# Dizzy-cell/HOUV

Measured on AMD Instinct MI355X. Metric: registration pairs/sec (2048-pt partial pairs), higher is better.
Workload: dtype f32; 1 GPU; HOUV solve_model, 2048x2048-pt pairs, batch 256/GPU, K=64 restarts x 200 Adam iterations + retry stages (BASELINE configs[1]); pairs_per_gpu=256, points=2048, kernel=64, iters=200, icp_refine=False, parallelism=dp1 (pair shards, one RCCL all-gather of [steps*P,12] per rank)

## Files before the change

houv_amd/_lib.py:

```python
import ctypes
import os

import torch

_HERE = os.path.dirname(os.path.abspath(__file__))
LIB_PATH = os.environ.get("HOUV_HIP_LIB") or os.path.join(_HERE, "lib", "libhouv_hip.so")
ABI_VERSION = 2

_c_f = ctypes.c_void_p
_int = ctypes.c_int
_dbl = ctypes.c_double
_flt = ctypes.c_float

_SIGNATURES = {
    "houv_abi_version": (ctypes.c_int, []),
    "houv_last_error": (ctypes.c_char_p, []),
    "houv_build_id": (ctypes.c_char_p, []),
    "houv_debug_set": (ctypes.c_int, [ctypes.c_char_p, ctypes.c_longlong]),
    "houv_chamfer_forward": (ctypes.c_int, [_c_f, _c_f, _int, _int, _int, _c_f, _c_f, _c_f, _c_f, _c_f]),
    "houv_chamfer_backward": (ctypes.c_int, [_c_f, _c_f, _int, _int, _int, _c_f, _c_f, _c_f, _c_f, _c_f, _c_f, _c_f]),
    "houv_kabsch": (ctypes.c_int, [_c_f, _c_f, _c_f, _int, _int, _c_f, _c_f, _c_f]),
    "houv_solve_iterate": (ctypes.c_int, [_c_f, _c_f, _int, _int, _int, _int, _c_f, _int, _int, _int, _int, _int, _int,
                                          _int, _int, _dbl, _dbl, _dbl, _dbl, _flt, _c_f, _c_f, _c_f, _c_f, _c_f, _c_f,
                                          _c_f]),
    "houv_solve_iterate_large": (ctypes.c_int, [_c_f, _c_f, _int, _int, _int, _int, _c_f, _int, _int, _int, _int, _int, _int,
                                                _int, _int, _dbl, _dbl, _dbl, _dbl, _flt, _c_f, _c_f, _c_f, _c_f, _c_f, _c_f,
                                                _c_f]),
    "houv_solve_iterate_pruned": (ctypes.c_int, [_c_f, _c_f, _int, _int, _int, _int, _c_f, _int, _int, _int, _int, _int,
                                                 _int, _int, _int, _dbl, _dbl, _dbl, _dbl, _flt, _c_f, _c_f, _c_f, _c_f,
                                                 _c_f, _c_f, _c_f, _int, _int, _c_f]),
    "houv_solve_variant": (ctypes.c_int, [_int, _int, _int, ctypes.POINTER(ctypes.c_int), ctypes.POINTER(ctypes.c_int),
                                          ctypes.POINTER(ctypes.c_int)]),
    "houv_solve_lds_bytes": (ctypes.c_longlong, [_int, _int, _int]),
    "houv_kd_sort": (ctypes.c_int, [_c_f, _int, _int, _int, _int, _c_f, _c_f, _c_f]),
    "houv_icp_refine": (ctypes.c_int, [_c_f, _c_f, _int, _int, _int, _c_f, _flt, _int, _flt, _flt, _c_f, _c_f, _c_f, _c_f, _c_f]),
    "houv_knn": (ctypes.c_int, [_c_f, _int, _int, _int, _c_f, _c_f]),
    "houv_edgeconv1": (ctypes.c_int, [_c_f, _c_f, _int, _int, _int, _c_f, _c_f, _c_f, _c_f, _c_f]),
    "houv_max_over_k": (ctypes.c_int, [_c_f, ctypes.c_longlong, _int, _int, _c_f, _int, _c_f]),
    "houv_gemm_f32": (ctypes.c_int, [_c_f, _c_f, _c_f, _int, _int, _int, _int, _int, _int, _int, _int, _int] +
                      [ctypes.c_longlong] * 6 + [_flt, _c_f, _c_f, _c_f, _int, ctypes.c_longlong, ctypes.c_longlong,
                                                 _int, _c_f]),
    "houv_attention_f32": (ctypes.c_int, [_c_f, _c_f, _c_f, _c_f, _int, _int, _int, _int, _int, _int, _int, _int, _int] +
                           [ctypes.c_longlong] * 4 + [_flt, _c_f]),
    "houv_layernorm": (ctypes.c_int, [_c_f, ctypes.c_longlong, _int, _c_f, _c_f, _flt, _c_f, _c_f, _c_f]),
    "houv_softmax_rows": (ctypes.c_int, [_c_f, ctypes.c_longlong, _int, _c_f]),
    "houv_softmax_corr": (ctypes.c_int, [_c_f, _int, _int, _int, _c_f, _c_f, _c_f]),
    "houv_furthest_point_sample": (ctypes.c_int, [_c_f, _int, _int, _int, _c_f, _c_f]),
    "houv_knn_cross": (ctypes.c_int, [_c_f, _c_f, _int, _int, _int, _int, _c_f, _c_f, _c_f]),
# ... 41 lines not shown
        fn.restype = res
        fn.argtypes = args
    if lib.houv_abi_version() != ABI_VERSION:
        raise HouvHipError(f"libhouv_hip.so ABI {lib.houv_abi_version()} != expected {ABI_VERSION}")
    _lib = lib
    return lib


def solve_variant(N, M, pruned=False, with_mode=False):
    b, q, m = ctypes.c_int(0), ctypes.c_int(0), ctypes.c_int(0)
    check(load().houv_solve_variant(int(N), int(M), int(bool(pruned)), ctypes.byref(b), ctypes.byref(q), ctypes.byref(m)),
          "houv_solve_variant")
    return (b.value, q.value, m.value) if with_mode else (b.value, q.value)


def build_id():
    return load().houv_build_id().decode()


def debug_set(name, value):
    check(load().houv_debug_set(name.encode(), int(value)), "houv_debug_set")


def last_error():
    return load().houv_last_error().decode("utf-8", "replace")


def check(ok, what):
    if ok != 1:
        raise HouvHipError(f"{what} failed: {last_error()}")
# ... 33 lines not shown
```

houv_amd/csrc/capi.hip:

```cpp
#include <stdarg.h>
#include <string.h>

#include "../../include/houv_hip.h"
#include "houv_common.h"

namespace houv {

static thread_local char g_err[512] = "";

void set_error(const char* fmt, ...) {
  va_list ap;
  va_start(ap, fmt);
  vsnprintf(g_err, sizeof(g_err), fmt, ap);
  va_end(ap);
  fprintf(stderr, "[houv_hip] %s\n", g_err);
}

DebugKnobs g_debug;

namespace {

__global__ void pose_kernel(const float* __restrict__ params, int n, int angle_base, int trans_mode,
                            float* __restrict__ R, float* __restrict__ T) {
  const int i = blockIdx.x * blockDim.x + threadIdx.x;
// ... 25 lines not shown
}

extern "C" int houv_abi_version(void) { return HOUV_ABI_VERSION; }

extern "C" const char* houv_last_error(void) { return houv::g_err; }

extern "C" int houv_debug_set(const char* name, long long value) {
  using namespace houv;
  const struct { const char* name; std::atomic<int>* knob; long long lo, hi, step; } ints[] = {
      {"solve_predict", &g_debug.pred_mode, 0, 2, 1}, {"knn_split", &g_debug.knn_split, 0, 1, 1},
      {"attn_split", &g_debug.attn_split, 0, 1, 1},   {"gemm_split", &g_debug.gemm_split, 0, 6, 3}};
  if (name && !strcmp(name, "solve_stats")) {
    g_debug.stats = (unsigned long long)value;
    return 1;
  }
  for (const auto& k : ints)
    if (name && !strcmp(name, k.name) && value >= k.lo && value <= k.hi && value % k.step == 0) {
      *k.knob = (int)value;
      return 1;
    }
  set_error("houv_debug_set: unknown switch or value out of range: %s = %lld", name ? name : "(null)", value);
  return 0;
}

#ifndef HOUV_BUILD_ID
#define HOUV_BUILD_ID "unknown"
#endif
extern "C" const char* houv_build_id(void) { return HOUV_BUILD_ID; }

extern "C" int houv_pose_forward(const float* params, int n, int angle_base, int trans_mode, const float* src, int N,
// ... 18 lines not shown
```

houv_amd/csrc/houv_common.h:

```cpp
#pragma once
#include <hip/hip_runtime.h>
#include <stdint.h>
#include <stdio.h>

#include <atomic>

#include "houv_math.h"

namespace houv {

constexpr int kWave = 64;
constexpr int kSub = 32;
constexpr int kTrk = 16;

void set_error(const char* fmt, ...);
struct SolveCommon;
__attribute__((visibility("hidden"))) int solve_check_args(const char* who, const SolveCommon& a, int use_views);
inline bool check_launch(const char* what) {
  hipError_t e = hipGetLastError();
  if (e != hipSuccess) {
    set_error("%s: %s", what, hipGetErrorString(e));
    return false;
  }
  return true;
}

struct DebugKnobs {
  std::atomic<int> pred_mode{0};
  std::atomic<unsigned long long> stats{0ull};
  std::atomic<int> knn_split{1};
  std::atomic<int> attn_split{1};
  std::atomic<int> gemm_split{6};
};
extern DebugKnobs g_debug;

template <int MET>
__device__ __forceinline__ float metric_sqdist(float dx, float dy, float dz) {
  if constexpr (MET == 0) return __builtin_fmaf(dz, dz, __builtin_fmaf(dy, dy, dx * dx));
  else if constexpr (MET == 1) return __builtin_fmaf(dz, dz, dy * dy);
  else if constexpr (MET == 2) return __builtin_fmaf(dz, dz, dx * dx);
  else return __builtin_fmaf(dy, dy, dx * dx);
}

__device__ __forceinline__ float min3f(float a, float b, float c) {
// ... 67 lines not shown
```

houv_amd/csrc/houv_math.h:

```cpp
#pragma once
#include <math.h>

#if defined(__HIPCC__)
#define HOUV_HD __host__ __device__
#else
#define HOUV_HD
#endif

namespace houv {

constexpr float kPiF = 3.14159274101257324f;

enum TransMode { kTransHouv = 0, kTransSolve = 1 };

HOUV_HD inline float tsqrt(float x) { return sqrtf(x); }
HOUV_HD inline double tsqrt(double x) { return sqrt(x); }

struct Pose {
  float R[9];
  float T[3];
  float u[3], inv_vnorm, sin_t, cos_t, chat[3], inv_cnorm, sigma, a, s;
};

HOUV_HD inline void pose_forward(const float p[8], int angle_base, int trans_mode, Pose& o) {
// ... 222 lines not shown
#pragma unroll
    for (int i = 0; i < 3; ++i) Ts[i] = stale[(m * 12 + 9 + i) * stride];
    term_travel(Rs, Ts, R, T, def_now, radius, d_s, t_s);
    const bool s0 = (stale_bits >> m) & 1u, s1 = (stale_bits >> (4 + m)) & 1u;
    const float d0 = s0 ? d_s : d_f, d1 = s1 ? d_s : d_f;
    const float t0 = s0 ? t_s : t_f, t1 = s1 ? t_s : t_f;
    const float c0 = cd[2 * m], c1 = cd[2 * m + 1];
    const float dd = d0 + d1;
    const float slack = dd + kTermRel * (fabsf(c0) + fabsf(c1) + dd) + kTermAbs +
                        kTermMoveErr * (2.0f * radius + tn + 0.5f * (t0 + t1));
    const unsigned drop1 = (c0 + slack < c1) ? (0x10u << m) : 0u;
    const unsigned drop0 = (c1 + slack < c0) ? (1u << m) : 0u;
    need &= ~(drop0 | drop1);
  }
  return need;
}

template <typename T>
HOUV_HD inline void svd3x3(const T H[9], T U[9], T S[3], T V[9]) {
  T B[9];
  for (int i = 0; i < 9; ++i) { B[i] = H[i]; V[i] = (i % 4 == 0) ? (T)1 : (T)0; }
  const int P[3] = {0, 0, 1}, Qi[3] = {1, 2, 2};
  for (int sweep = 0; sweep < 12; ++sweep) {
    T off = 0;
    for (int r = 0; r < 3; ++r) {
      const int p = P[r], q = Qi[r];
      const T a = B[0 * 3 + p] * B[0 * 3 + p] + B[1 * 3 + p] * B[1 * 3 + p] + B[2 * 3 + p] * B[2 * 3 + p];
      const T b = B[0 * 3 + q] * B[0 * 3 + q] + B[1 * 3 + q] * B[1 * 3 + q] + B[2 * 3 + q] * B[2 * 3 + q];
      const T g = B[0 * 3 + p] * B[0 * 3 + q] + B[1 * 3 + p] * B[1 * 3 + q] + B[2 * 3 + p] * B[2 * 3 + q];
      const T eps2 = sizeof(T) == 4 ? (T)1e-14 : (T)1e-31;
// ... 74 lines not shown
```

houv_amd/csrc/houv_sweep.h:

```cpp
#pragma once
#include "houv_common.h"

namespace houv {

typedef float houv_f4v __attribute__((ext_vector_type(4)));
typedef const houv_f4v __attribute__((address_space(3))) * lds_f4;

__device__ __forceinline__ int tid_x() {
  int t = threadIdx.x;
  asm volatile("" : "+v"(t));
  return t;
}
typedef __amdgpu_buffer_rsrc_t buf_t;
__device__ __forceinline__ buf_t make_buf(const void* base, int bytes) {
  return __builtin_amdgcn_make_buffer_rsrc(const_cast<void*>(base), (short)0, bytes, 0x00020000);
}

template <int Q, int NMET>
__device__ __forceinline__ void sweep_tile(const float4* __restrict__ rp, const float (&qx)[Q], const float (&qy)[Q],
                                           const float (&qz)[Q], const float (&in)[Q][NMET], float (&out)[Q][NMET]) {
#pragma unroll
  for (int j = 0; j < kTrk; j += 2) {
    const float4 a = rp[j], c = rp[j + 1];
    asm volatile("" ::"v"(a.w), "v"(c.w));
// ... 170 lines not shown

constexpr int kNnRec = 8;

__device__ __forceinline__ unsigned select_mask(unsigned long long lanes, unsigned a, unsigned b) {
  unsigned r;
  asm("v_cndmask_b32_e64 %0, %1, %2, %3" : "=v"(r) : "v"(a), "v"(b), "s"(lanes));
  return r;
}

__device__ __forceinline__ unsigned lowest_bit_or_m1(unsigned x) {
  unsigned r;
  asm("v_ffbl_b32_e32 %0, %1" : "=v"(r) : "v"(x));
  return r;
}

template <int NMET>
__device__ __forceinline__ void gather_tile_min(unsigned xa, float cx, float cy, float cz, const float (&cb)[NMET],
                                                float (&ta)[NMET], float (&tb)[NMET]) {
  constexpr int kBatch = 4, kHalf = kSub / 2;
  static_assert(kSub == 32 && kHalf == kTrk, "two 256-B tracking units of 16 slots");
  auto fetch = [&](float4 (&r)[kBatch], int i0) {
#pragma unroll
    for (int u = 0; u < kBatch; u += 2) {
      lds_f4 p = (lds_f4)(size_t)(xa ^ ((unsigned)((i0 + u / 2) & (kHalf - 1)) << 4));
      const houv_f4v v0 = p[0], v1 = p[kHalf];
      r[u] = make_float4(v0.x, v0.y, v0.z, v0.w);
      r[u + 1] = make_float4(v1.x, v1.y, v1.z, v1.w);
    }
  };
  auto eval2 = [&](const float4 a, const float4 c, const float (&in)[NMET], float (&t)[NMET]) {
    const float ax = a.x - cx, ay = a.y - cy, az = a.z - cz;
    const float bx = c.x - cx, by = c.y - cy, bz = c.z - cz;
    if constexpr (NMET == 4) {
      const float axx = ax * ax, ayy = ay * ay, bxx = bx * bx, byy = by * by;
      const float a3 = __builtin_fmaf(ay, ay, axx), b3 = __builtin_fmaf(by, by, bxx);
      const float a1 = __builtin_fmaf(az, az, ayy), b1 = __builtin_fmaf(bz, bz, byy);
      const float a2 = __builtin_fmaf(az, az, axx), b2 = __builtin_fmaf(bz, bz, bxx);
      const float a0 = __builtin_fmaf(az, az, a3), b0 = __builtin_fmaf(bz, bz, b3);
      t[0] = min3f(in[0], a0, b0);
      t[1] = min3f(in[1], a1, b1);
      t[2] = min3f(in[2], a2, b2);
      t[3] = min3f(in[3], a3, b3);
    } else {
      t[0] = min3f(in[0], metric_sqdist<0>(ax, ay, az), metric_sqdist<0>(bx, by, bz));
    }
  };
  float inf[NMET];
#pragma unroll
  for (int m = 0; m < NMET; ++m) inf[m] = INFINITY;
  auto eval = [&](float4 (&r)[kBatch], bool first) {
#pragma unroll
    for (int u = 0; u < kBatch; ++u) asm volatile("" ::"v"(r[u].x), "v"(r[u].y), "v"(r[u].z), "v"(r[u].w));
    static_assert(kBatch == 4, "a batch = two slots x two units");
    if (first) {
      eval2(r[0], r[2], cb, ta);
      eval2(r[1], r[3], inf, tb);
    } else {
      eval2(r[0], r[2], ta, ta);
      eval2(r[1], r[3], tb, tb);
    }
  };
  float4 ra[kBatch], rb[kBatch];
  fetch(ra, 0);
#pragma unroll
  for (int i0 = 0; i0 < kHalf; i0 += kBatch) {
    fetch(rb, i0 + kBatch / 2);
    eval(ra, i0 == 0);
    if (i0 + kBatch < kHalf) fetch(ra, i0 + kBatch);
    eval(rb, false);
  }
}

__device__ __forceinline__ void take_units(float ta, float tb, int unit0, float& cb, int& ct) {
  const unsigned long long la = __builtin_amdgcn_ballot_w64(ta < cb), lb = __builtin_amdgcn_ballot_w64(tb < ta);
  ct = (int)select_mask(lb, select_mask(la, (unsigned)ct, (unsigned)unit0), (unsigned)unit0 + 1u);
  cb = __uint_as_float(select_mask(lb, __float_as_uint(ta), __float_as_uint(tb)));
}

template <int BLOCK, int Q, int NMET>
__device__ __forceinline__ void prune_masks(const float4* __restrict__ refs, const float4* __restrict__ boxes, int ntile,
                                            const float (&qx)[Q], const float (&qy)[Q], const float (&qz)[Q],
                                            buf_t ws, int prev_off, int count, unsigned need,
                                            unsigned long long (&un)[Q]) {
  float ub[Q][NMET];
#pragma unroll
  for (int k = 0; k < Q; ++k) {
    const bool ok = pt_index<BLOCK>(k) < count;
    unsigned w0 = 0u, w1 = 0u;
    const int voff = tid_x() * kNnRec, soff = prev_off + pt_base<BLOCK>(k) * kNnRec;
    if (ok) {
      if constexpr (NMET == 4) {
        const auto r = __builtin_amdgcn_raw_buffer_load_b64(ws, voff, soff, 0);
        w0 = r[0]; w1 = r[1];
      } else {
        w0 = __builtin_amdgcn_raw_buffer_load_b32(ws, voff, soff, 0);
      }
    }
    { const float4 r = refs[w0 & 0xffffu]; ub[k][0] = metric_sqdist<0>(r.x - qx[k], r.y - qy[k], r.z - qz[k]); }
    if constexpr (NMET == 4) {
      { const float4 r = refs[w0 >> 16]; ub[k][1] = metric_sqdist<1>(r.x - qx[k], r.y - qy[k], r.z - qz[k]); }
      { const float4 r = refs[w1 & 0xffffu]; ub[k][2] = metric_sqdist<2>(r.x - qx[k], r.y - qy[k], r.z - qz[k]); }
      { const float4 r = refs[w1 >> 16]; ub[k][3] = metric_sqdist<3>(r.x - qx[k], r.y - qy[k], r.z - qz[k]); }
    }
#pragma unroll
    for (int m = 0; m < NMET; ++m)
      ub[k][m] = (ok && ((need >> m) & 1u)) ? (ub[k][m] * 1.00001f + 1e-30f) : -1.f;
  }
  unsigned alo[Q], ahi[Q];
#pragma unroll
  for (int k = 0; k < Q; ++k) alo[k] = ahi[k] = 0u;
  auto test = [&](const float4 lo, const float4 hi, unsigned (&acc)[Q]) {
#pragma unroll
    for (int k = 0; k < Q; ++k) {
      const float dx = qx[k] - __builtin_amdgcn_fmed3f(qx[k], lo.x, hi.x);
      const float dy = qy[k] - __builtin_amdgcn_fmed3f(qy[k], lo.y, hi.y);
      const float dz = qz[k] - __builtin_amdgcn_fmed3f(qz[k], lo.z, hi.z);
      unsigned long long in;
      if constexpr (NMET == 4) {
        const float xx = dx * dx, yy = dy * dy;
        const float s3 = __builtin_fmaf(dy, dy, xx), s1 = __builtin_fmaf(dz, dz, yy), s2 = __builtin_fmaf(dz, dz, xx);
        const float s0 = __builtin_fmaf(dz, dz, s3);
        in = __builtin_amdgcn_ballot_w64(s0 <= ub[k][0]) | __builtin_amdgcn_ballot_w64(s1 <= ub[k][1]) |
             __builtin_amdgcn_ballot_w64(s2 <= ub[k][2]) | __builtin_amdgcn_ballot_w64(s3 <= ub[k][3]);
      } else {
        in = __builtin_amdgcn_ballot_w64(__builtin_fmaf(dz, dz, __builtin_fmaf(dy, dy, dx * dx)) <= ub[k][0]);
      }
      acc[k] = shift_in_mask(acc[k], in);
    }
  };
  auto run = [&](int t_first, int t_last, unsigned (&acc)[Q]) {
    float4 lo = boxes[2 * t_first], hi = boxes[2 * t_first + 1];
    for (int t = t_first; t >= t_last; --t) {
      const int tn = t > 0 ? t - 1 : 0;
      const float4 nlo = boxes[2 * tn], nhi = boxes[2 * tn + 1];
      test(lo, hi, acc);
      lo = nlo; hi = nhi;
    }
  };
  if (ntile > 32) run(ntile - 1, 32, ahi);
  run((ntile < 32 ? ntile : 32) - 1, 0, alo);
#pragma unroll
  for (int k = 0; k < Q; ++k) un[k] = ((unsigned long long)ahi[k] << 32) | alo[k];
}

struct SortedStage {
  unsigned short* order;
  int* hist;
};

__device__ __forceinline__ unsigned& w_slot(float4* cloud, int q) { return reinterpret_cast<unsigned*>(cloud + q)[3]; }

template <int BLOCK, int Q, int NMET, int TS = 0>
__device__ __forceinline__ void pruned_sweep_sorted(const float4* __restrict__ refs, const float4* __restrict__ boxes, int ntile,
                                                    const float4* __restrict__ qarr, float4* wlo, float4* whi,
                                                    const float (&qx)[Q], const float (&qy)[Q], const float (&qz)[Q],
                                                    buf_t ws, int prev_off, int count, unsigned need, int rot,
                                                    const SortedStage& st, float4* __restrict__ res, float (&best)[Q][NMET],
                                                    int (&btile)[Q][NMET], unsigned long long* __restrict__ stats) {
  static_assert(BLOCK % 64 == 0 && BLOCK >= 128, "whole waves; thread 64 resets the block counter");
  const int tid = tid_x(), lane = tid & 63;
  unsigned long long un[Q];
  prune_masks<BLOCK, Q, NMET>(refs, boxes, ntile, qx, qy, qz, ws, prev_off, count, need, un);
  int len[Q], rnk[Q];
#pragma unroll
  for (int k = 0; k < Q; ++k) {
    const int q = pt_index<BLOCK>(k);
    len[k] = __popcll(un[k]);
    rnk[k] = 0;
    if (q < count) {
      w_slot(wlo, q) = (unsigned)un[k];
      w_slot(whi, q) = (unsigned)(un[k] >> 32);
      rnk[k] = atomicAdd(&st.hist[64 - len[k]], 1);
    }
  }
  __syncthreads();
  const int bin_c = st.hist[lane];
  const int bin_incl = wave_incl_scan_dpp(bin_c);
  const int base64 = __builtin_amdgcn_readlane(bin_incl, 63);
  if (tid == 64) st.hist[130] = 0;
#pragma unroll
  for (int k = 0; k < Q; ++k) {
    const int q = pt_index<BLOCK>(k);
    const int bin = 64 - len[k];
    const int base = __builtin_amdgcn_ds_bpermute((bin & 63) << 2, bin_incl - bin_c);
    if (q < count) st.order[(bin == 64 ? base64 : base) + rnk[k]] = (unsigned short)q;
  }
  __syncthreads();
  if (tid < 65) st.hist[tid] = 0;
  const int nblk = (count + 63) >> 6;
  int asked = 0, nsteps = 0;
  for (;;) {
    int b = 0;
    if (lane == 0) b = atomicAdd(&st.hist[130], 1);
    b = __builtin_amdgcn_readfirstlane(b);
    if (b >= nblk) break;
    const int e = b * 64 + lane;
    const bool valid = e < count;
    const int q = st.order[valid ? e : count - 1];
    unsigned long long mm = valid ? (((unsigned long long)w_slot(whi, q) << 32) | w_slot(wlo, q)) : 0ull;
    const int cap = __builtin_amdgcn_readfirstlane(__popcll(mm));
    const float4 qp = qarr[q];
    float cb[NMET];
    int ct[NMET];
#pragma unroll
    for (int m = 0; m < NMET; ++m) { cb[m] = INFINITY; ct[m] = 0; }
    asked += __popcll(mm);
    nsteps += cap;
    const unsigned xbase = (unsigned)(size_t)(lds_f4)refs + (((unsigned)rot & 15u) << 4);
    int t = 0;
#pragma unroll 1
    for (int s = 0; s < cap; ++s) {
      const unsigned nxt = min(lowest_bit_or_m1((unsigned)mm), lowest_bit_or_m1((unsigned)(mm >> 32)) | 32u);
      t = max(t, (int)nxt);
      mm &= mm - 1ull;
#pragma unroll
      for (int h = 0; h < (1 << TS); ++h) {
        const int ts = (t << TS) | h;
        const unsigned xa = xbase + (unsigned)ts * (kSub * 16u);
        float ta[NMET], tb[NMET];
        gather_tile_min<NMET>(xa, qp.x, qp.y, qp.z, cb, ta, tb);
#pragma unroll
        for (int m = 0; m < NMET; ++m) take_units(ta[m], tb[m], 2 * ts, cb[m], ct[m]);
      }
    }
    if (valid) {
      if constexpr (NMET == 4) {
        res[q] = make_float4(cb[0], cb[1], cb[2], cb[3]);
        w_slot(wlo, q) = (unsigned)ct[0] | ((unsigned)ct[1] << 8) | ((unsigned)ct[2] << 16) | ((unsigned)ct[3] << 24);
      } else {
        res[q].x = cb[0];
        w_slot(wlo, q) = (unsigned)ct[0];
      }
    }
  }
  if (stats) {
    asked = wave_incl_scan_dpp(asked);
    if (lane == 63) atomicAdd(&stats[0], (unsigned long long)asked);
    if (lane == 0) {
      atomicAdd(&stats[1], (unsigned long long)nsteps);
      atomicAdd(&stats[2], 1ull);
    }
  }
  __syncthreads();
#pragma unroll
  for (int k = 0; k < Q; ++k) {
    const int q = pt_index<BLOCK>(k);
    const bool ok = q < count && len[k] > 0;
    const int qq = ok ? q : 0;
    const unsigned tl = w_slot(wlo, qq);
// ... 3 lines not shown
      btile[k][0] = ok ? (int)(tl & 255u) : 0; btile[k][1] = ok ? (int)((tl >> 8) & 255u) : 0;
      btile[k][2] = ok ? (int)((tl >> 16) & 255u) : 0; btile[k][3] = ok ? (int)(tl >> 24) : 0;
    } else {
      const float r = res[qq].x;
      best[k][0] = ok ? r : INFINITY;
      btile[k][0] = ok ? (int)(tl & 255u) : 0;
    }
  }
}

template <int BLOCK, int Q, int TS = 0>
__device__ __forceinline__ void tile_boxes(const float (&x)[Q], const float (&y)[Q], const float (&z)[Q], int count,
                                           int ntile, float4* __restrict__ box) {
  constexpr int kTile = kSub << TS;
  static_assert(kTile <= 64, "a tile's owners must sit in one wave");
#pragma unroll
  for (int k = 0; k < Q; ++k) {
    float lx = INFINITY, ly = INFINITY, lz = INFINITY, hx = -INFINITY, hy = -INFINITY, hz = -INFINITY;
    if (pt_index<BLOCK>(k) < count) {
      lx = fminf(lx, x[k]); ly = fminf(ly, y[k]); lz = fminf(lz, z[k]);
      hx = fmaxf(hx, x[k]); hy = fmaxf(hy, y[k]); hz = fmaxf(hz, z[k]);
    }
#pragma unroll
    for (int o = 1; o < kTile; o <<= 1) {
      lx = fminf(lx, __shfl_xor(lx, o, 64)); ly = fminf(ly, __shfl_xor(ly, o, 64)); lz = fminf(lz, __shfl_xor(lz, o, 64));
      hx = fmaxf(hx, __shfl_xor(hx, o, 64)); hy = fmaxf(hy, __shfl_xor(hy, o, 64)); hz = fmaxf(hz, __shfl_xor(hz, o, 64));
    }
    const int t = pt_index<BLOCK>(k) / kTile;
    if ((tid_x() % kTile) == 0 && t < ntile) {
      box[2 * t] = make_float4(lx, ly, lz, 0.f);
      box[2 * t + 1] = make_float4(hx, hy, hz, 0.f);
    }
  }
}

}
```

houv_amd/csrc/solve.hip:

```cpp
#include <stddef.h>
#include <stdlib.h>

#include "../../include/houv_hip.h"
#include "houv_common.h"
#include "houv_solve.h"

namespace houv {
namespace {

struct SolveArgs : SolveCommon {
  short* nn_ws;
  int ws_valid;
  int ws_stride;
  int pred_mode;
  unsigned long long* stats;
};

constexpr int kRescanBatch = 4;
constexpr int kRefresh = 4;
constexpr int kTermMaxAge = 0;

struct Smem {
  float4* tgt;
  float4* mov;
  double* state;
  double* adam;
  float* pose;
  float* acc;
  float* red;
  unsigned* hist;
// ... 296 lines not shown
  const int pair = inst / a.K;
  const buf_t src = make_buf(a.src + (size_t)pair * N * 3, N * 12);
  const float* __restrict__ tgt = a.tgt + (size_t)pair * M * 3;
  const int npad = (N + kPad - 1) / kPad * kPad, mpad = (M + kPad - 1) / kPad * kPad;
  const float4 pad4 = make_float4(INFINITY, INFINITY, INFINITY, 0.f);

  for (int j = tid; j < mpad; j += BLOCK) sm.tgt[j] = (j < M) ? make_float4(tgt[j * 3], tgt[j * 3 + 1], tgt[j * 3 + 2], 0.f) : pad4;
  for (int j = N + tid; j < npad; j += BLOCK) sm.mov[j] = pad4;
  if (tid < 24) sm.state[tid] = a.state[(size_t)inst * 24 + tid];
  for (int j = tid; j < kHistBins; j += BLOCK) sm.hist[j] = 0u;
  if constexpr (PRUNE) {
    if (tid < 132) sm.st.hist[tid] = 0;
  }
  int hrot = 0;
  __syncthreads();
  const int rot = tid & (kSub - 1);
  buf_t ws = src;
  const int ws_b = 0, ws_a = a.ws_stride * kNnRec;
  float4* ws_res = nullptr;
  if constexpr (PRUNE) {
    ws = make_buf(a.nn_ws + (size_t)inst * 16 * a.ws_stride, 32 * a.ws_stride);
    ws_res = reinterpret_cast<float4*>(a.nn_ws + ((size_t)inst * 16 + 8) * a.ws_stride);
    float tx0[Q], ty0[Q], tz0[Q];
#pragma unroll
    for (int k = 0; k < Q; ++k) {
      const int i = pt_index<BLOCK>(k);
      const float4 v = (i < M) ? sm.tgt[i] : make_float4(0.f, 0.f, 0.f, 0.f);
      tx0[k] = v.x; ty0[k] = v.y; tz0[k] = v.z;
    }
    tile_boxes<BLOCK, Q, TS>(tx0, ty0, tz0, M, mpad / kPad, sm.tbox);
  }
// ... 34 lines not shown
    if (tid == 0) {
      float r2 = 0.f;
      for (int w = 0; w < BLOCK / 64; ++w) r2 = fmaxf(r2, sm.red[w]);
      sm.anchor[kTermAnchorFloats] = sqrtf(r2) * 1.000001f;
    }
  }

  unsigned long long clk0 = 0ull, rt0 = 0ull;
  if (a.stats) {
    clk0 = __builtin_amdgcn_s_memtime();
    rt0 = __builtin_amdgcn_s_memrealtime();
  }
  constexpr int NW = BLOCK / 64;
  constexpr unsigned kAllMet = (1u << NMET) - 1u;
  unsigned pred_a = kAllMet;
  float* red_a = sm.red + ((size_t)1 * NW + (tid >> 6)) * kRedStride;
  float* red_b = sm.red + ((size_t)0 * NW + (tid >> 6)) * kRedStride;
#pragma unroll 1
  for (int it = 0; it < a.n_iters; ++it) {
    if (a.pred_mode == 1) pred_a = 0u;
    const bool allgrad = a.pred_mode == 2 || ((PRUNE != 0) && (((a.steps_done + it) % kRefresh) == 0 || (a.ws_valid == 0 && it == 0)));
    unsigned need_a = kAllMet, need_b = kAllMet;
    if constexpr (PRUNE != 0) {
      const unsigned w = (unsigned)__builtin_amdgcn_readfirstlane(sm.ctl[0]);
      need_b = w & kAllMet;
      need_a = (w >> 4) & kAllMet;
    }
    const unsigned grad_a = (allgrad ? kAllMet : (pred_a | ~need_b)) & need_a;
    {
      float sx[Q], sy[Q], sz[Q], mx[Q], my[Q], mz[Q];
      float R[9], T[3];
      load_rt(fresh_lds(sm.pose), R, T);
#pragma unroll
      for (int k = 0; k < Q; ++k) {
        const int i = pt_index<BLOCK>(k);
        const bool ok = i < N;
        load_src_point<BLOCK>(src, k, N, sx[k], sy[k], sz[k]);
        move_point(R, T, sx[k], sy[k], sz[k], mx[k], my[k], mz[k]);
        if (ok) sm.mov[i] = make_float4(mx[k], my[k], mz[k], 0.f);
      }
      __syncthreads();
      bool pruned_now = false;
      float best[Q][NMET];
      int btile[Q][NMET];
      if constexpr (PRUNE) {
        tile_boxes<BLOCK, Q, TS>(mx, my, mz, N, npad / kPad, sm.mbox);
        pruned_now = (a.ws_valid != 0) || (it > 0);
      }
      if (need_a != 0u) {
        if (pruned_now) {
          if constexpr (PRUNE != 0)
            pruned_sweep_sorted<BLOCK, Q, NMET, TS>(sm.tgt, sm.tbox, mpad / kPad, sm.mov, sm.tgt, sm.mov, mx, my, mz, ws, ws_a, N,
                                                need_a, rot, sm.st, ws_res, best, btile, a.stats);
        } else {
          sweep<Q, NMET>(sm.tgt, mpad / kTrk, mx, my, mz, best, btile);
          if (a.stats && (tid & 63) == 0) atomicAdd(&a.stats[3], 1ull);
        }
        unsigned sel[NMET];
        select_all<BLOCK, Q, NMET>(sm, best, N, a.k_full, a.k_view, need_a, hrot, sel);
        park_sqrt_sums<BLOCK, Q, NMET>(best, sel, need_a, red_a);
        park_grad_sums<BLOCK, Q, NMET, 1, PRUNE != 0>(sm, sm.tgt, mx, my, mz, best, btile, sel, grad_a, N, sx, sy, sz, red_a, ws,
                                                     ws_a);
      }
      __syncthreads();
      final_sums<BLOCK, NMET>(sm, 1, true, grad_a, need_a);
    }
    unsigned pick_a;
    {
      float tx[Q], ty[Q], tz[Q];
#pragma unroll
      for (int k = 0; k < Q; ++k) {
        const int i = pt_index<BLOCK>(k);
        const float4 v = (i < M) ? sm.tgt[i] : make_float4(0.f, 0.f, 0.f, 0.f);
        tx[k] = v.x; ty[k] = v.y; tz[k] = v.z;
      }
      const bool pruned_now = (PRUNE != 0) && ((a.ws_valid != 0) || (it > 0));
      auto pick_winners = [&]() {
        __syncthreads();
        final_sums<BLOCK, NMET>(sm, 0, true, 0u, need_b);
        __syncthreads();
        pick_a = picked_direction<NMET>(sm, fresh(a.k_full), fresh(a.k_view));
        return (allgrad ? kAllMet : (~pick_a & kAllMet)) & need_b;
      };
      unsigned grad_b = 0u;
      if (need_b != 0u) {
        float best[Q][NMET];
        int btile[Q][NMET];
        if (pruned_now) {
          if constexpr (PRUNE != 0)
            pruned_sweep_sorted<BLOCK, Q, NMET, TS>(sm.mov, sm.mbox, npad / kPad, sm.tgt, sm.tgt, sm.mov, tx, ty, tz, ws, ws_b, M,
                                                need_b, rot, sm.st, ws_res, best, btile, a.stats);
        } else {
          sweep<Q, NMET>(sm.mov, npad / kTrk, tx, ty, tz, best, btile);
          if (a.stats && (tid & 63) == 0) atomicAdd(&a.stats[3], 1ull);
        }
        unsigned sel[NMET];
        select_all<BLOCK, Q, NMET>(sm, best, M, a.k_full, a.k_view, need_b, hrot, sel);
        park_sqrt_sums<BLOCK, Q, NMET>(best, sel, need_b, red_b);
        grad_b = pick_winners();
        park_grad_sums<BLOCK, Q, NMET, 0, PRUNE != 0>(sm, sm.mov, tx, ty, tz, best, btile, sel, grad_b, M, tx, ty, tz, red_b, ws,
                                                     ws_b);
      } else {
        pick_winners();
      }
      const unsigned miss = pick_a & ~grad_a & kAllMet;
      if (miss) {
        if (miss & 1u) repair_direction_a<BLOCK, Q, 0>(sm, src, N, mpad, a.k_full, hrot, red_a);
        if constexpr (NMET == 4) {
          if (miss & 2u) repair_direction_a<BLOCK, Q, 1>(sm, src, N, mpad, a.k_view, hrot, red_a);
          if (miss & 4u) repair_direction_a<BLOCK, Q, 2>(sm, src, N, mpad, a.k_view, hrot, red_a);
          if (miss & 8u) repair_direction_a<BLOCK, Q, 3>(sm, src, N, mpad, a.k_view, hrot, red_a);
        }
      }
      __syncthreads();
      final_sums<BLOCK, NMET>(sm, 0, false, grad_b, kAllMet);
      if (miss) final_sums<BLOCK, NMET>(sm, 1, false, miss, kAllMet);
    }
    pred_a = pick_a;
    static_assert(NMET * kAccN <= 64, "final_sums runs on the scalar tail's wave");
    __builtin_amdgcn_wave_barrier();

    if (kAdamTid != 0 && tid == kAdamTid && it + 1 < a.n_iters) {
      const int step = a.steps_done + it + 2;
      const AdamScalars asc = adam_scalars(step, fresh(a.lr), fresh(a.beta1), fresh(a.beta2));
      sm.adam[(step & 1) * 2 + 0] = asc.step_size;
      sm.adam[(step & 1) * 2 + 1] = asc.bc2_sqrt;
// ... 107 lines not shown
  else if (mx <= 256) { b = 256; q = 1; }
  else if (mx <= 512) { b = 256; q = 2; }
  else if (mx <= 768) { b = 256; q = 3; }
  else if (mx <= 1024) { b = 256; q = 4; }
  else if (mx <= 1536) { b = 512; q = 3; }
  else if (mx <= 2048) { b = 512; q = 4; }
  else if (mx <= 3072) { b = 1024; q = 3; }
  else { b = 1024; q = 4; }
  if (block) *block = b;
  if (points_per_lane) *points_per_lane = q;
  constexpr int kPrunedMinPoints = 257;
  if (prune_mode) *prune_mode = (!pruned || mx < kPrunedMinPoints) ? 0 : (mx > 2048) ? 3 : 2;
  return 1;
}

extern "C" long long houv_solve_lds_bytes(int N, int M, int pruned) {
  using namespace houv;
  int block = 0, q = 0, mode = 0;
  if (!houv_solve_variant(N, M, pruned, &block, &q, &mode)) return -1;
  return (long long)smem_bytes(N, M, block, mode, q);
}

int houv::solve_check_args(const char* who, const SolveCommon& a, int use_views) {
  const int P = a.P, N = a.N, M = a.M;
  if (P < 0 || N <= 0 || M <= 0 || a.K <= 0 || a.n_iters <= 0 || a.steps_done < 0 || a.angle_base < 0 || a.angle_base > 3 ||
      a.trans_mode < 0 || a.trans_mode > 1) {
    set_error("%s: bad argument P=%d N=%d M=%d K=%d n_iters=%d steps_done=%d base=%d trans_mode=%d", who, P, N, M, a.K,
              a.n_iters, a.steps_done, a.angle_base, a.trans_mode);
    return 0;
  }
// ... 9 lines not shown
  }
  if ((long long)P * a.K > 0x7fffffffLL) {
    set_error("%s: too many hypotheses", who);
    return 0;
  }
  return 2;
}

static int solve_dispatch(const houv::SolveCommon& c, int use_views, short* nn_ws, int ws_valid, int ws_stride, bool prune,
                          void* stream, const char* who) {
  using namespace houv;
  const int ok = solve_check_args(who, c, use_views);
  if (ok < 2) return ok;
  const int N = c.N, M = c.M;
  SolveArgs a{c, nn_ws, ws_valid, ws_stride, g_debug.pred_mode.load(),
              reinterpret_cast<unsigned long long*>(g_debug.stats.load())};
  hipStream_t s = (hipStream_t)stream;
  const int mx = N > M ? N : M;
  int block = 0, q = 0, mode = 0;
  if (!houv_solve_variant(N, M, prune ? 1 : 0, &block, &q, &mode)) return 0;
  if (prune && (!nn_ws || ws_stride < mx || (ws_stride & 7))) {
    set_error("%s: pruned mode needs a workspace of 16 x ws_stride int16 per hypothesis, ws_stride >= max(N,M) and a multiple of 8", who);
    return 0;
  }
  if (prune && ((uintptr_t)nn_ws & 15)) {
    set_error("%s: the pruned-mode workspace must be 16-byte aligned", who);
    return 0;
  }
  if (prune && ws_valid < 0) {
    a.ws_valid = 0;
    mode = 0;
// ... 40 lines not shown
```

include/houv_hip.h:

```cpp
#ifndef HOUV_HIP_H_
#define HOUV_HIP_H_

#include <stdint.h>

#ifdef __cplusplus
extern "C" {
#endif

#define HOUV_ABI_VERSION 2

int houv_abi_version(void);

const char* houv_last_error(void);

const char* houv_build_id(void);

int houv_debug_set(const char* name, long long value);

int houv_chamfer_forward(const float* xyz1, const float* xyz2, int B, int N, int M,
                         float* dist1, float* dist2, int32_t* idx1, int32_t* idx2, void* stream);

int houv_chamfer_backward(const float* xyz1, const float* xyz2, int B, int N, int M,
                          const float* graddist1, const float* graddist2,
                          const int32_t* idx1, const int32_t* idx2,
// ... 19 lines not shown
                              float* out_grad, float* out_cd,
                              int16_t* nn_ws, int ws_valid, int ws_stride, void* stream);

#define HOUV_LARGE_MAX_POINTS 16384
int houv_solve_iterate_large(const float* src, const float* tgt, int P, int N, int M, int K,
                             double* state, int steps_done, int n_iters,
                             int angle_base, int trans_mode, int use_views, int f64_params,
                             int k_full, int k_view,
                             double lr, double beta1, double beta2, double eps, float loss_scale,
                             float* out_score, float* out_loss, float* out_R, float* out_T,
                             float* out_grad, float* out_cd, void* stream);

int houv_solve_variant(int N, int M, int pruned, int* block, int* points_per_lane, int* prune_mode);

long long houv_solve_lds_bytes(int N, int M, int pruned);

int houv_kd_sort(const float* xyz, int P, int N, int leaf, int rule, float* out, int32_t* order_or_null, void* stream);

int houv_icp_refine(const float* src, const float* tgt, int P, int N, int M, const float* init_or_null,
                    float max_correspondence_distance, int max_iteration, float relative_fitness,
                    float relative_rmse, float* out_T, float* out_fitness, float* out_rmse, int32_t* out_iters,
                    void* stream);


int houv_knn(const float* xyz, int B, int N, int k, int32_t* idx, void* stream);

int houv_edgeconv1(const float* xyz, const int32_t* idx, int B, int N, int k, const float* W, const float* scale,
                   const float* shift, float* out, void* stream);

int houv_max_over_k(const float* act, long long npts, int k, int C, float* out, int ldo, void* stream);
// ... 81 lines not shown
```

Baseline: 195.3 pairs/s.

## Specialize pruned sweep by needed metric subset to skip unused distance terms

Adds compile-time metric-subset variants of the pruned nearest-neighbour walk and prune-mask builder, chosen at runtime from the per-direction 'need' mask through a constexpr cost table. Only the needed metrics' distances, mins, ballots and tile updates are computed, so pruned sweeps that need fewer of the four metrics avoid wasted ALU work. It also replaces __shfl_xor in the box reduction with raw ds_bpermute, derives the LDS rotation from the thread id, and adds an optional debug walk histogram. The switch dispatch duplicates code, which grows the kernel and may raise register pressure, and the empty asm pins are there to steer scheduling.

```diff
diff --git a/houv_amd/_lib.py b/houv_amd/_lib.py
--- a/houv_amd/_lib.py
+++ b/houv_amd/_lib.py
@@ -32,6 +32,7 @@
     "houv_solve_variant": (ctypes.c_int, [_int, _int, _int, ctypes.POINTER(ctypes.c_int), ctypes.POINTER(ctypes.c_int),
                                           ctypes.POINTER(ctypes.c_int)]),
     "houv_solve_lds_bytes": (ctypes.c_longlong, [_int, _int, _int]),
+    "houv_solve_walk_variant": (ctypes.c_int, [_int]),
     "houv_kd_sort": (ctypes.c_int, [_c_f, _int, _int, _int, _int, _c_f, _c_f, _c_f]),
     "houv_icp_refine": (ctypes.c_int, [_c_f, _c_f, _int, _int, _int, _c_f, _flt, _int, _flt, _flt, _c_f, _c_f, _c_f, _c_f, _c_f]),
     "houv_knn": (ctypes.c_int, [_c_f, _int, _int, _int, _c_f, _c_f]),
@@ -103,6 +104,13 @@
     return (b.value, q.value, m.value) if with_mode else (b.value, q.value)
 
 
+def solve_walk_variant(need):
+    v = load().houv_solve_walk_variant(int(need))
+    if v < 0:
+        raise HouvHipError(f"houv_solve_walk_variant failed: {last_error()}")
+    return v
+
+
 def build_id():
     return load().houv_build_id().decode()
 
diff --git a/houv_amd/csrc/capi.hip b/houv_amd/csrc/capi.hip
--- a/houv_amd/csrc/capi.hip
+++ b/houv_amd/csrc/capi.hip
@@ -63,6 +63,10 @@
     g_debug.stats = (unsigned long long)value;
     return 1;
   }
+  if (name && !strcmp(name, "solve_walk_hist")) {
+    g_debug.walk_hist = (unsigned long long)value;
+    return 1;
+  }
   for (const auto& k : ints)
     if (name && !strcmp(name, k.name) && value >= k.lo && value <= k.hi && value % k.step == 0) {
       *k.knob = (int)value;
diff --git a/houv_amd/csrc/houv_common.h b/houv_amd/csrc/houv_common.h
--- a/houv_amd/csrc/houv_common.h
+++ b/houv_amd/csrc/houv_common.h
@@ -28,6 +28,7 @@
 struct DebugKnobs {
   std::atomic<int> pred_mode{0};
   std::atomic<unsigned long long> stats{0ull};
+  std::atomic<unsigned long long> walk_hist{0ull};
   std::atomic<int> knn_split{1};
   std::atomic<int> attn_split{1};
   std::atomic<int> gemm_split{6};
diff --git a/houv_amd/csrc/houv_math.h b/houv_amd/csrc/houv_math.h
--- a/houv_amd/csrc/houv_math.h
+++ b/houv_amd/csrc/houv_math.h
@@ -260,6 +260,32 @@
     need &= ~(drop0 | drop1);
   }
   return need;
+}
+
+constexpr int kWalkSets[] = {6, 11, 12, 13, 15};
+constexpr int kNumWalkSets = (int)(sizeof(kWalkSets) / sizeof(kWalkSets[0]));
+constexpr int walk_step_cost(unsigned mset) {
+  const int k0 = (int)(mset & 1u), k1 = (int)((mset >> 1) & 1u), k2 = (int)((mset >> 2) & 1u), k3 = (int)((mset >> 3) & 1u);
+  return 16 * (2 * (k0 + k1 + k2 + ((k0 | k3) ? 1 : 0)) + 2 * k1 + (k0 + k1 + k2 + k3)) + 5 * (k0 + k1 + k2 + k3);
+}
+constexpr bool walk_instantiated(unsigned mset) {
+  for (int i = 0; i < kNumWalkSets; ++i)
+    if ((unsigned)kWalkSets[i] == mset) return true;
+  return false;
+}
+constexpr unsigned walk_variant(unsigned need) {
+  unsigned best = 15u;
+  for (int i = 0; i < kNumWalkSets; ++i) {
+    const unsigned s = (unsigned)kWalkSets[i];
+    if ((s & need) == need && walk_step_cost(s) < walk_step_cost(best)) best = s;
+  }
+  return best;
+}
+static_assert(walk_instantiated(15u) && walk_variant(15u) == 15u && walk_step_cost(15u) == 16 * 14 + 20, "today's code is a variant");
+constexpr unsigned long long walk_variant_table() {
+  unsigned long long t = 0ull;
+  for (unsigned n = 0; n < 16u; ++n) t |= (unsigned long long)walk_variant(n) << (4 * n);
+  return t;
 }
 
 template <typename T>
diff --git a/houv_amd/csrc/houv_sweep.h b/houv_amd/csrc/houv_sweep.h
--- a/houv_amd/csrc/houv_sweep.h
+++ b/houv_amd/csrc/houv_sweep.h
@@ -1,4 +1,6 @@
 #pragma once
+#include <type_traits>
+
 #include "houv_common.h"
 
 namespace houv {
@@ -208,7 +210,7 @@
   return r;
 }
 
-template <int NMET>
+template <int NMET, int MSET = (1 << NMET) - 1>
 __device__ __forceinline__ void gather_tile_min(unsigned xa, float cx, float cy, float cz, const float (&cb)[NMET],
                                                 float (&ta)[NMET], float (&tb)[NMET]) {
   constexpr int kBatch = 4, kHalf = kSub / 2;
@@ -231,10 +233,10 @@
       const float a1 = __builtin_fmaf(az, az, ayy), b1 = __builtin_fmaf(bz, bz, byy);
       const float a2 = __builtin_fmaf(az, az, axx), b2 = __builtin_fmaf(bz, bz, bxx);
       const float a0 = __builtin_fmaf(az, az, a3), b0 = __builtin_fmaf(bz, bz, b3);
-      t[0] = min3f(in[0], a0, b0);
-      t[1] = min3f(in[1], a1, b1);
-      t[2] = min3f(in[2], a2, b2);
-      t[3] = min3f(in[3], a3, b3);
+      if constexpr ((MSET & 1) != 0) t[0] = min3f(in[0], a0, b0);
+      if constexpr ((MSET & 2) != 0) t[1] = min3f(in[1], a1, b1);
+      if constexpr ((MSET & 4) != 0) t[2] = min3f(in[2], a2, b2);
+      if constexpr ((MSET & 8) != 0) t[3] = min3f(in[3], a3, b3);
     } else {
       t[0] = min3f(in[0], metric_sqdist<0>(ax, ay, az), metric_sqdist<0>(bx, by, bz));
     }
@@ -254,14 +256,17 @@
       eval2(r[1], r[3], tb, tb);
     }
   };
+  constexpr bool kPin = NMET == 4 && MSET != (1 << NMET) - 1;
   float4 ra[kBatch], rb[kBatch];
   fetch(ra, 0);
 #pragma unroll
   for (int i0 = 0; i0 < kHalf; i0 += kBatch) {
     fetch(rb, i0 + kBatch / 2);
     eval(ra, i0 == 0);
+    if constexpr (kPin) asm volatile("" : "+v"(xa));
     if (i0 + kBatch < kHalf) fetch(ra, i0 + kBatch);
     eval(rb, false);
+    if constexpr (kPin) asm volatile("" : "+v"(xa));
   }
 }
 
@@ -271,7 +276,7 @@
   cb = __uint_as_float(select_mask(lb, __float_as_uint(ta), __float_as_uint(tb)));
 }
 
-template <int BLOCK, int Q, int NMET>
+template <int BLOCK, int Q, int NMET, int MSET = (1 << NMET) - 1>
 __device__ __forceinline__ void prune_masks(const float4* __restrict__ refs, const float4* __restrict__ boxes, int ntile,
                                             const float (&qx)[Q], const float (&qy)[Q], const float (&qz)[Q],
                                             buf_t ws, int prev_off, int count, unsigned need,
@@ -290,15 +295,15 @@
         w0 = __builtin_amdgcn_raw_buffer_load_b32(ws, voff, soff, 0);
       }
     }
-    { const float4 r = refs[w0 & 0xffffu]; ub[k][0] = metric_sqdist<0>(r.x - qx[k], r.y - qy[k], r.z - qz[k]); }
+    if constexpr ((MSET & 1) != 0) { const float4 r = refs[w0 & 0xffffu]; ub[k][0] = metric_sqdist<0>(r.x - qx[k], r.y - qy[k], r.z - qz[k]); }
     if constexpr (NMET == 4) {
-      { const float4 r = refs[w0 >> 16]; ub[k][1] = metric_sqdist<1>(r.x - qx[k], r.y - qy[k], r.z - qz[k]); }
-      { const float4 r = refs[w1 & 0xffffu]; ub[k][2] = metric_sqdist<2>(r.x - qx[k], r.y - qy[k], r.z - qz[k]); }
-      { const float4 r = refs[w1 >> 16]; ub[k][3] = metric_sqdist<3>(r.x - qx[k], r.y - qy[k], r.z - qz[k]); }
+      if constexpr ((MSET & 2) != 0) { const float4 r = refs[w0 >> 16]; ub[k][1] = metric_sqdist<1>(r.x - qx[k], r.y - qy[k], r.z - qz[k]); }
+      if constexpr ((MSET & 4) != 0) { const float4 r = refs[w1 & 0xffffu]; ub[k][2] = metric_sqdist<2>(r.x - qx[k], r.y - qy[k], r.z - qz[k]); }
+      if constexpr ((MSET & 8) != 0) { const float4 r = refs[w1 >> 16]; ub[k][3] = metric_sqdist<3>(r.x - qx[k], r.y - qy[k], r.z - qz[k]); }
     }
 #pragma unroll
     for (int m = 0; m < NMET; ++m)
-      ub[k][m] = (ok && ((need >> m) & 1u)) ? (ub[k][m] * 1.00001f + 1e-30f) : -1.f;
+      if ((MSET >> m) & 1) ub[k][m] = (ok && ((need >> m) & 1u)) ? (ub[k][m] * 1.00001f + 1e-30f) : -1.f;
   }
   unsigned alo[Q], ahi[Q];
 #pragma unroll
@@ -314,8 +319,11 @@
         const float xx = dx * dx, yy = dy * dy;
         const float s3 = __builtin_fmaf(dy, dy, xx), s1 = __builtin_fmaf(dz, dz, yy), s2 = __builtin_fmaf(dz, dz, xx);
         const float s0 = __builtin_fmaf(dz, dz, s3);
-        in = __builtin_amdgcn_ballot_w64(s0 <= ub[k][0]) | __builtin_amdgcn_ballot_w64(s1 <= ub[k][1]) |
-             __builtin_amdgcn_ballot_w64(s2 <= ub[k][2]) | __builtin_amdgcn_ballot_w64(s3 <= ub[k][3]);
+        in = 0ull;
+        if constexpr ((MSET & 1) != 0) in |= __builtin_amdgcn_ballot_w64(s0 <= ub[k][0]);
+        if constexpr ((MSET & 2) != 0) in |= __builtin_amdgcn_ballot_w64(s1 <= ub[k][1]);
+        if constexpr ((MSET & 4) != 0) in |= __builtin_amdgcn_ballot_w64(s2 <= ub[k][2]);
+        if constexpr ((MSET & 8) != 0) in |= __builtin_amdgcn_ballot_w64(s3 <= ub[k][3]);
       } else {
         in = __builtin_amdgcn_ballot_w64(__builtin_fmaf(dz, dz, __builtin_fmaf(dy, dy, dx * dx)) <= ub[k][0]);
       }
@@ -344,17 +352,38 @@
 
 __device__ __forceinline__ unsigned& w_slot(float4* cloud, int q) { return reinterpret_cast<unsigned*>(cloud + q)[3]; }
 
+template <typename F>
+__device__ __forceinline__ void walk_dispatch(unsigned mset, F&& f) {
+#define HOUV_WALK_CASE(S)                                                          \
+  case S:                                                                          \
+    if constexpr (walk_instantiated(S)) f(std::integral_constant<int, S>{});       \
+    break;
+  switch (mset) {
+    HOUV_WALK_CASE(1) HOUV_WALK_CASE(2) HOUV_WALK_CASE(3) HOUV_WALK_CASE(4) HOUV_WALK_CASE(5) HOUV_WALK_CASE(6) HOUV_WALK_CASE(7)
+    HOUV_WALK_CASE(8) HOUV_WALK_CASE(9) HOUV_WALK_CASE(10) HOUV_WALK_CASE(11) HOUV_WALK_CASE(12) HOUV_WALK_CASE(13) HOUV_WALK_CASE(14)
+    default: f(std::integral_constant<int, 15>{}); break;
+  }
+#undef HOUV_WALK_CASE
+}
+
 template <int BLOCK, int Q, int NMET, int TS = 0>
 __device__ __forceinline__ void pruned_sweep_sorted(const float4* __restrict__ refs, const float4* __restrict__ boxes, int ntile,
                                                     const float4* __restrict__ qarr, float4* wlo, float4* whi,
                                                     const float (&qx)[Q], const float (&qy)[Q], const float (&qz)[Q],
-                                                    buf_t ws, int prev_off, int count, unsigned need, int rot,
+                                                    buf_t ws, int prev_off, int count, unsigned need,
                                                     const SortedStage& st, float4* __restrict__ res, float (&best)[Q][NMET],
-                                                    int (&btile)[Q][NMET], unsigned long long* __restrict__ stats) {
+                                                    int (&btile)[Q][NMET], unsigned long long* __restrict__ stats,
+                                                    unsigned long long* __restrict__ walk_hist) {
   static_assert(BLOCK % 64 == 0 && BLOCK >= 128, "whole waves; thread 64 resets the block counter");
   const int tid = tid_x(), lane = tid & 63;
   unsigned long long un[Q];
-  prune_masks<BLOCK, Q, NMET>(refs, boxes, ntile, qx, qy, qz, ws, prev_off, count, need, un);
+  if constexpr (NMET == 4) {
+    walk_dispatch((unsigned)(walk_variant_table() >> (4u * need)) & 15u, [&](auto mset) {
+      prune_masks<BLOCK, Q, NMET, decltype(mset)::value>(refs, boxes, ntile, qx, qy, qz, ws, prev_off, count, need, un);
+    });
+  } else {
+    prune_masks<BLOCK, Q, NMET>(refs, boxes, ntile, qx, qy, qz, ws, prev_off, count, need, un);
+  }
   int len[Q], rnk[Q];
 #pragma unroll
   for (int k = 0; k < Q; ++k) {
@@ -383,50 +412,57 @@
   if (tid < 65) st.hist[tid] = 0;
   const int nblk = (count + 63) >> 6;
   int asked = 0, nsteps = 0;
-  for (;;) {
-    int b = 0;
-    if (lane == 0) b = atomicAdd(&st.hist[130], 1);
-    b = __builtin_amdgcn_readfirstlane(b);
-    if (b >= nblk) break;
-    const int e = b * 64 + lane;
-    const bool valid = e < count;
-    const int q = st.order[valid ? e : count - 1];
-    unsigned long long mm = valid ? (((unsigned long long)w_slot(whi, q) << 32) | w_slot(wlo, q)) : 0ull;
-    const int cap = __builtin_amdgcn_readfirstlane(__popcll(mm));
-    const float4 qp = qarr[q];
-    float cb[NMET];
-    int ct[NMET];
-#pragma unroll
-    for (int m = 0; m < NMET; ++m) { cb[m] = INFINITY; ct[m] = 0; }
-    asked += __popcll(mm);
-    nsteps += cap;
-    const unsigned xbase = (unsigned)(size_t)(lds_f4)refs + (((unsigned)rot & 15u) << 4);
-    int t = 0;
+  auto walk_blocks = [&](auto mset) {
+    constexpr int MSET = decltype(mset)::value;
+    for (;;) {
+      int b = 0;
+      if (lane == 0) b = atomicAdd(&st.hist[130], 1);
+      b = __builtin_amdgcn_readfirstlane(b);
+      if (b >= nblk) break;
+      const int e = b * 64 + lane;
+      const bool valid = e < count;
+      const int q = st.order[valid ? e : count - 1];
+      unsigned long long mm = valid ? (((unsigned long long)w_slot(whi, q) << 32) | w_slot(wlo, q)) : 0ull;
+      const int cap = __builtin_amdgcn_readfirstlane(__popcll(mm));
+      const float4 qp = qarr[q];
+      float cb[NMET];
+      int ct[NMET];
+#pragma unroll
+      for (int m = 0; m < NMET; ++m) { cb[m] = INFINITY; ct[m] = 0; }
+      asked += __popcll(mm);
+      nsteps += cap;
+      const unsigned xbase = (unsigned)(size_t)(lds_f4)refs + (((unsigned)tid_x() & 15u) << 4);
+      int t = 0;
 #pragma unroll 1
-    for (int s = 0; s < cap; ++s) {
-      const unsigned nxt = min(lowest_bit_or_m1((unsigned)mm), lowest_bit_or_m1((unsigned)(mm >> 32)) | 32u);
-      t = max(t, (int)nxt);
-      mm &= mm - 1ull;
-#pragma unroll
-      for (int h = 0; h < (1 << TS); ++h) {
-        const int ts = (t << TS) | h;
-        const unsigned xa = xbase + (unsigned)ts * (kSub * 16u);
-        float ta[NMET], tb[NMET];
-        gather_tile_min<NMET>(xa, qp.x, qp.y, qp.z, cb, ta, tb);
-#pragma unroll
-        for (int m = 0; m < NMET; ++m) take_units(ta[m], tb[m], 2 * ts, cb[m], ct[m]);
-      }
-    }
-    if (valid) {
-      if constexpr (NMET == 4) {
-        res[q] = make_float4(cb[0], cb[1], cb[2], cb[3]);
-        w_slot(wlo, q) = (unsigned)ct[0] | ((unsigned)ct[1] << 8) | ((unsigned)ct[2] << 16) | ((unsigned)ct[3] << 24);
-      } else {
-        res[q].x = cb[0];
-        w_slot(wlo, q) = (unsigned)ct[0];
-      }
-    }
-  }
+      for (int s = 0; s < cap; ++s) {
+        const unsigned nxt = min(lowest_bit_or_m1((unsigned)mm), lowest_bit_or_m1((unsigned)(mm >> 32)) | 32u);
+        t = max(t, (int)nxt);
+        mm &= mm - 1ull;
+#pragma unroll
+        for (int h = 0; h < (1 << TS); ++h) {
+          const int ts = (t << TS) | h;
+          const unsigned xa = xbase + (unsigned)ts * (kSub * 16u);
+          float ta[NMET], tb[NMET];
+          gather_tile_min<NMET, MSET>(xa, qp.x, qp.y, qp.z, cb, ta, tb);
+#pragma unroll
+          for (int m = 0; m < NMET; ++m)
+            if ((MSET >> m) & 1) take_units(ta[m], tb[m], 2 * ts, cb[m], ct[m]);
+        }
+      }
+      if (valid) {
+        if constexpr (NMET == 4) {
+          res[q] = make_float4(cb[0], cb[1], cb[2], cb[3]);
+          w_slot(wlo, q) = (unsigned)ct[0] | ((unsigned)ct[1] << 8) | ((unsigned)ct[2] << 16) | ((unsigned)ct[3] << 24);
+        } else {
+          res[q].x = cb[0];
+          w_slot(wlo, q) = (unsigned)ct[0];
+        }
+      }
+    }
+  };
+  if constexpr (NMET == 4) walk_dispatch((unsigned)(walk_variant_table() >> (4u * need)) & 15u, walk_blocks);
+  else walk_blocks(std::integral_constant<int, 1>{});
+  if (walk_hist && lane == 0) atomicAdd(&walk_hist[need & 15u], 1ull);
   if (stats) {
     asked = wave_incl_scan_dpp(asked);
     if (lane == 63) atomicAdd(&stats[0], (unsigned long long)asked);
@@ -460,6 +496,8 @@
                                            int ntile, float4* __restrict__ box) {
   constexpr int kTile = kSub << TS;
   static_assert(kTile <= 64, "a tile's owners must sit in one wave");
+  const int lane4 = tid_x() << 2;
+  auto shfl_xor = [&](float v, int o) { return __int_as_float(__builtin_amdgcn_ds_bpermute((lane4 ^ (o << 2)) & 252, __float_as_int(v))); };
 #pragma unroll
   for (int k = 0; k < Q; ++k) {
     float lx = INFINITY, ly = INFINITY, lz = INFINITY, hx = -INFINITY, hy = -INFINITY, hz = -INFINITY;
@@ -469,8 +507,8 @@
     }
 #pragma unroll
     for (int o = 1; o < kTile; o <<= 1) {
-      lx = fminf(lx, __shfl_xor(lx, o, 64)); ly = fminf(ly, __shfl_xor(ly, o, 64)); lz = fminf(lz, __shfl_xor(lz, o, 64));
-      hx = fmaxf(hx, __shfl_xor(hx, o, 64)); hy = fmaxf(hy, __shfl_xor(hy, o, 64)); hz = fmaxf(hz, __shfl_xor(hz, o, 64));
+      lx = fminf(lx, shfl_xor(lx, o)); ly = fminf(ly, shfl_xor(ly, o)); lz = fminf(lz, shfl_xor(lz, o));
+      hx = fmaxf(hx, shfl_xor(hx, o)); hy = fmaxf(hy, shfl_xor(hy, o)); hz = fmaxf(hz, shfl_xor(hz, o));
     }
     const int t = pt_index<BLOCK>(k) / kTile;
     if ((tid_x() % kTile) == 0 && t < ntile) {
diff --git a/houv_amd/csrc/solve.hip b/houv_amd/csrc/solve.hip
--- a/houv_amd/csrc/solve.hip
+++ b/houv_amd/csrc/solve.hip
@@ -14,6 +14,7 @@
   int ws_stride;
   int pred_mode;
   unsigned long long* stats;
+  unsigned long long* walk_hist;
 };
 
 constexpr int kRescanBatch = 4;
@@ -340,7 +341,6 @@
   }
   int hrot = 0;
   __syncthreads();
-  const int rot = tid & (kSub - 1);
   buf_t ws = src;
   const int ws_b = 0, ws_a = a.ws_stride * kNnRec;
   float4* ws_res = nullptr;
@@ -405,15 +405,14 @@
   constexpr int NW = BLOCK / 64;
   constexpr unsigned kAllMet = (1u << NMET) - 1u;
   unsigned pred_a = kAllMet;
-  float* red_a = sm.red + ((size_t)1 * NW + (tid >> 6)) * kRedStride;
-  float* red_b = sm.red + ((size_t)0 * NW + (tid >> 6)) * kRedStride;
+  auto red_row = [&](int dir) { return sm.red + ((size_t)dir * NW + (tid_x() >> 6)) * kRedStride; };
 #pragma unroll 1
   for (int it = 0; it < a.n_iters; ++it) {
     if (a.pred_mode == 1) pred_a = 0u;
     const bool allgrad = a.pred_mode == 2 || ((PRUNE != 0) && (((a.steps_done + it) % kRefresh) == 0 || (a.ws_valid == 0 && it == 0)));
     unsigned need_a = kAllMet, need_b = kAllMet;
     if constexpr (PRUNE != 0) {
-      const unsigned w = (unsigned)__builtin_amdgcn_readfirstlane(sm.ctl[0]);
+      const unsigned w = (unsigned)__builtin_amdgcn_readfirstlane(*reinterpret_cast<const int*>(fresh_lds(reinterpret_cast<const float*>(sm.ctl))));
       need_b = w & kAllMet;
       need_a = (w >> 4) & kAllMet;
     }
@@ -442,15 +441,15 @@
         if (pruned_now) {
           if constexpr (PRUNE != 0)
             pruned_sweep_sorted<BLOCK, Q, NMET, TS>(sm.tgt, sm.tbox, mpad / kPad, sm.mov, sm.tgt, sm.mov, mx, my, mz, ws, ws_a, N,
-                                                need_a, rot, sm.st, ws_res, best, btile, a.stats);
+                                                need_a, sm.st, ws_res, best, btile, a.stats, fresh(a.walk_hist));
         } else {
           sweep<Q, NMET>(sm.tgt, mpad / kTrk, mx, my, mz, best, btile);
           if (a.stats && (tid & 63) == 0) atomicAdd(&a.stats[3], 1ull);
         }
         unsigned sel[NMET];
         select_all<BLOCK, Q, NMET>(sm, best, N, a.k_full, a.k_view, need_a, hrot, sel);
-        park_sqrt_sums<BLOCK, Q, NMET>(best, sel, need_a, red_a);
-        park_grad_sums<BLOCK, Q, NMET, 1, PRUNE != 0>(sm, sm.tgt, mx, my, mz, best, btile, sel, grad_a, N, sx, sy, sz, red_a, ws,
+        park_sqrt_sums<BLOCK, Q, NMET>(best, sel, need_a, red_row(1));
+        park_grad_sums<BLOCK, Q, NMET, 1, PRUNE != 0>(sm, sm.tgt, mx, my, mz, best, btile, sel, grad_a, N, sx, sy, sz, red_row(1), ws,
                                                      ws_a);
       }
       __syncthreads();
@@ -480,27 +479,27 @@
         if (pruned_now) {
           if constexpr (PRUNE != 0)
             pruned_sweep_sorted<BLOCK, Q, NMET, TS>(sm.mov, sm.mbox, npad / kPad, sm.tgt, sm.tgt, sm.mov, tx, ty, tz, ws, ws_b, M,
-                                                need_b, rot, sm.st, ws_res, best, btile, a.stats);
+                                                need_b, sm.st, ws_res, best, btile, a.stats, fresh(a.walk_hist));
         } else {
           sweep<Q, NMET>(sm.mov, npad / kTrk, tx, ty, tz, best, btile);
           if (a.stats && (tid & 63) == 0) atomicAdd(&a.stats[3], 1ull);
         }
         unsigned sel[NMET];
         select_all<BLOCK, Q, NMET>(sm, best, M, a.k_full, a.k_view, need_b, hrot, sel);
-        park_sqrt_sums<BLOCK, Q, NMET>(best, sel, need_b, red_b);
+        park_sqrt_sums<BLOCK, Q, NMET>(best, sel, need_b, red_row(0));
         grad_b = pick_winners();
-        park_grad_sums<BLOCK, Q, NMET, 0, PRUNE != 0>(sm, sm.mov, tx, ty, tz, best, btile, sel, grad_b, M, tx, ty, tz, red_b, ws,
+        park_grad_sums<BLOCK, Q, NMET, 0, PRUNE != 0>(sm, sm.mov, tx, ty, tz, best, btile, sel, grad_b, M, tx, ty, tz, red_row(0), ws,
                                                      ws_b);
       } else {
         pick_winners();
       }
       const unsigned miss = pick_a & ~grad_a & kAllMet;
       if (miss) {
-        if (miss & 1u) repair_direction_a<BLOCK, Q, 0>(sm, src, N, mpad, a.k_full, hrot, red_a);
+        if (miss & 1u) repair_direction_a<BLOCK, Q, 0>(sm, src, N, mpad, a.k_full, hrot, red_row(1));
         if constexpr (NMET == 4) {
-          if (miss & 2u) repair_direction_a<BLOCK, Q, 1>(sm, src, N, mpad, a.k_view, hrot, red_a);
-          if (miss & 4u) repair_direction_a<BLOCK, Q, 2>(sm, src, N, mpad, a.k_view, hrot, red_a);
-          if (miss & 8u) repair_direction_a<BLOCK, Q, 3>(sm, src, N, mpad, a.k_view, hrot, red_a);
+          if (miss & 2u) repair_direction_a<BLOCK, Q, 1>(sm, src, N, mpad, a.k_view, hrot, red_row(1));
+          if (miss & 4u) repair_direction_a<BLOCK, Q, 2>(sm, src, N, mpad, a.k_view, hrot, red_row(1));
+          if (miss & 8u) repair_direction_a<BLOCK, Q, 3>(sm, src, N, mpad, a.k_view, hrot, red_row(1));
         }
       }
       __syncthreads();
@@ -638,6 +637,14 @@
   return 1;
 }
 
+extern "C" int houv_solve_walk_variant(int need) {
+  if (need < 0 || need > 15) {
+    houv::set_error("houv_solve_walk_variant: the term mask of a direction is 0..15, got %d", need);
+    return -1;
+  }
+  return (int)houv::walk_variant((unsigned)need);
+}
+
 extern "C" long long houv_solve_lds_bytes(int N, int M, int pruned) {
   using namespace houv;
   int block = 0, q = 0, mode = 0;
@@ -677,7 +684,8 @@
   if (ok < 2) return ok;
   const int N = c.N, M = c.M;
   SolveArgs a{c, nn_ws, ws_valid, ws_stride, g_debug.pred_mode.load(),
-              reinterpret_cast<unsigned long long*>(g_debug.stats.load())};
+              reinterpret_cast<unsigned long long*>(g_debug.stats.load()),
+              reinterpret_cast<unsigned long long*>(g_debug.walk_hist.load())};
   hipStream_t s = (hipStream_t)stream;
   const int mx = N > M ? N : M;
   int block = 0, q = 0, mode = 0;
diff --git a/include/houv_hip.h b/include/houv_hip.h
--- a/include/houv_hip.h
+++ b/include/houv_hip.h
@@ -57,6 +57,8 @@
 int houv_solve_variant(int N, int M, int pruned, int* block, int* points_per_lane, int* prune_mode);
 
 long long houv_solve_lds_bytes(int N, int M, int pruned);
+
+int houv_solve_walk_variant(int need);
 
 int houv_kd_sort(const float* xyz, int P, int N, int leaf, int rule, float* out, int32_t* order_or_null, void* stream);
 
```

New measurement: 206.4 pairs/s (median of 6 runs). 1.06x the previous value.
